# pyro-ppl/pyro

Hardware: AMD Instinct MI355X
Metric: ELBO-grad steps/sec (SVI) (higher is better)
Workload: dtype f32; 1 GPU; BASELINE configs[1]: Bayesian logistic regression, plate=1000000, D=32, Trace_ELBO num_particles=64 per GPU (vectorised), AutoNormal, Adam; full SVI.step of SVI(model, guide, optim, loss), one hipGraph replay per step; parallelism=particles sharded x1, flat RCCL grad all-reduce

## Files before the change

### include/pyro_amd.h

```cpp
#ifndef PYRO_AMD_H
#define PYRO_AMD_H

#include <stddef.h>
#include <stdint.h>

#ifdef __cplusplus
extern "C" {
#endif

#define PA_ABI_VERSION 9

enum { PA_OK = 0, PA_ERR_INVALID = -1, PA_ERR_UNSUPPORTED = -2, PA_ERR_LAUNCH = -3 };

enum { PA_F32 = 0, PA_F64 = 1 };

enum {
  PA_DIST_NORMAL = 0,
  PA_DIST_BERNOULLI_LOGITS = 1,
  PA_DIST_HALF_CAUCHY = 2,
  PA_DIST_LOG_NORMAL = 3,
  PA_DIST_EXPONENTIAL = 4,
  PA_DIST_HALF_NORMAL = 5,
  PA_DIST_GAMMA = 6,
  PA_DIST_BETA = 7,
// ... 372 lines not shown
int pa_tall_wgrad(const float* G, const float* X, int64_t B, int64_t R, int64_t K, float* dW, float* db,
                  void* workspace, size_t workspace_bytes, pa_stream_t stream);
int pa_tall_linear_act(const float* G, int64_t B, int64_t R, const float* W, int64_t w_row_stride,
                       int64_t w_col_stride, int64_t C, const float* bias, const float* y_mul,
                       int sigmoid_out, float* Y, pa_stream_t stream);
int pa_tall_wgrad_act(const float* G, const float* X, const float* y_mul, int64_t B, int64_t R, int64_t K,
                      float* dW, float* db, void* workspace, size_t workspace_bytes, pa_stream_t stream);
int pa_tall_linear_path(int64_t B, int64_t R, int64_t C, int64_t w_row_stride, int64_t w_col_stride,
                        int g_aligned16, int ymul_aligned16, int w_aligned16);
int pa_tall_wgrad_path(int64_t B, int64_t R, int64_t K);

int pa_gamma_rsample(int dtype, void* out, void* d_alpha, pa_view2d alpha, int64_t rows, int64_t cols,
                     uint64_t seed, uint64_t offset, const uint64_t* offset_dev, pa_stream_t stream);
int pa_gamma_implicit_grad(int dtype, void* d_alpha, pa_view2d alpha, pa_view2d value, int64_t rows,
                           int64_t cols, pa_stream_t stream);

#define PA_CHAIN_SYNC_BYTES 64
int pa_chain_begin(pa_stream_t stream, void* sync_words, size_t sync_bytes);
int pa_chain_flush(void);
int pa_chain_end(int* launches, int* phases);
int pa_chain_pending(void);
int pa_chain_tune(int fuse_tail);
int pa_chain_fused_launches(void);
int pa_chain_debug_stamps(void* stamps32);

#define PA_RTC_MAX_POINTERS 384
int pa_rtc_compile(const char* source, const char* kernel_name, void** function_out);
int pa_rtc_compile_cached(const char* source, const char* kernel_name, const char* cache_file,
                          void** function_out, int* compiled_out);
int pa_rtc_version(int* hiprtc_major, int* hiprtc_minor, int* runtime_version);
void* pa_rtc_blocks_begin(void);
int pa_rtc_blocks_end(void* scope, int64_t* n_blocks_out);
int pa_rtc_blocks_free(void* scope);
int pa_rtc_launch(void* function, uint32_t grid, uint32_t block, const void* const* pointers,
                  int n_pointers, pa_stream_t stream);

size_t pa_mixture_workspace(int K, int64_t B);
int pa_mixture_fwd_bwd(int dtype, int dist, const void* x, int64_t N, int K, int64_t B, const void* a,
                       int64_t a_batch_stride, const void* p0, int64_t p0_stride, int64_t p0_batch_stride,
                       const void* p1, int64_t p1_stride, int64_t p1_batch_stride, void* workspace,
                       size_t workspace_bytes, double* out, pa_stream_t stream);

int pa_mixture_diag_normal_layout(int K, int D, int* kp_out, int* dd_out);
size_t pa_mixture_diag_normal_workspace(int K, int D, int64_t B);
int pa_mixture_diag_normal_fwd_bwd(int dtype, const void* x, int64_t N, int D, int K, int64_t B, const void* a,
                                   int64_t a_batch_stride, const void* loc, int64_t loc_stride_k,
// ... 59 lines not shown
```

### pyro_amd/_lib.py

```python
import ctypes
import os
from ctypes import (POINTER, Structure, c_char_p, c_double, c_int, c_int32, c_int64, c_size_t, c_uint32,
                    c_uint64, c_void_p)

_HERE = os.path.dirname(os.path.abspath(__file__))
LIB_PATH = os.path.join(_HERE, "lib", "libpyro_amd.so")

PA_OK, PA_ERR_INVALID, PA_ERR_UNSUPPORTED, PA_ERR_LAUNCH = 0, -1, -2, -3
PA_F32, PA_F64 = 0, 1
ABI_VERSION = 9

DIST_NORMAL = 0
DIST_BERNOULLI_LOGITS = 1
DIST_HALF_CAUCHY = 2
DIST_LOG_NORMAL = 3
DIST_EXPONENTIAL = 4
DIST_HALF_NORMAL = 5
DIST_GAMMA = 6
DIST_BETA = 7
DIST_POISSON = 8
DIST_BINOMIAL_LOGITS = 9
DIST_KL_NORMAL_LOC = 10
DIST_KL_NORMAL_SCALE = 11

# ... 280 lines not shown
                                c_void_p]),
    "pa_bow_workspace": (c_size_t, [c_int64, c_int64, c_int64]),
    "pa_bow_linear_fwd": (c_int, [c_void_p, c_void_p, c_void_p, c_int64, c_int64, c_int64, c_void_p,
                                  c_void_p, c_size_t, c_void_p]),
    "pa_bow_linear_bwd": (c_int, [c_void_p, c_void_p, c_int64, c_int64, c_int64, c_void_p, c_void_p,
                                  c_size_t, c_void_p]),
    "pa_bow_linear_fwd_act": (c_int, [c_void_p, c_void_p, c_void_p, c_int64, c_int64, c_int64, c_int, c_void_p,
                                      c_void_p, c_size_t, c_void_p]),
    "pa_bow_linear_bwd_act": (c_int, [c_void_p, c_void_p, c_void_p, c_int64, c_int64, c_int64, c_void_p,
                                      c_void_p, c_void_p, c_size_t, c_void_p]),
    "pa_tsgemm_tn_workspace": (c_size_t, [c_int64, c_int64, c_int64]),
    "pa_tsgemm_tn": (c_int, [c_void_p, c_void_p, c_int64, c_int64, c_int64, c_void_p, c_void_p, c_size_t,
                             c_void_p]),
    "pa_gamma_rsample": (c_int, [c_int, c_void_p, c_void_p, View2D, c_int64, c_int64, c_uint64, c_uint64,
                                 c_void_p, c_void_p]),
    "pa_gamma_implicit_grad": (c_int, [c_int, c_void_p, View2D, View2D, c_int64, c_int64, c_void_p]),
    "pa_chain_begin": (c_int, [c_void_p, c_void_p, c_size_t]),
    "pa_chain_flush": (c_int, []),
    "pa_chain_end": (c_int, [POINTER(c_int), POINTER(c_int)]),
    "pa_chain_pending": (c_int, []),
    "pa_chain_debug_stamps": (c_int, [c_void_p]),
    "pa_chain_tune": (c_int, [c_int]),
    "pa_chain_fused_launches": (c_int, []),
    "pa_adam_step_publish": (c_int, [c_int, c_void_p, c_void_p, c_void_p, c_void_p, c_int64,
                                     c_double, c_double, c_double, c_double, c_double, c_double,
                                     c_double, c_int, c_void_p, c_int, c_int, c_void_p, c_void_p,
                                     c_void_p, c_void_p, c_uint64, c_void_p]),
}

_lib = None


def exported_symbols():
    return sorted(_SIGNATURES)


def load(path=None):
    global _lib
    if _lib is not None:
        return _lib
    path = path or os.environ.get("PYRO_AMD_LIB", LIB_PATH)
    if not os.path.exists(path):
        raise RuntimeError(
            "pyro_amd: HIP extension %s not found. Build it with "
            "`python -m pyro_amd.csrc.build` (hipcc --offload-arch=gfx950). There is no CPU "
            "fallback." % path)
# ... 24 lines not shown
```

### pyro_amd/csrc/chain.hip

```cpp
#include "chain.h"
#include "glm_finalize.h"
#include "multisite_dev.h"
#include "optim_dev.h"
#include "site_tail.h"

namespace pa {

constexpr int CH_FIN = 0, CH_MULTI = 1, CH_MF = 2, CH_ADAM = 3, CH_PHASES = 4;
constexpr int CH_MF_SITES = 8;

struct MfArgs8 {
  int nsites;
  MfSiteDev s[CH_MF_SITES];
};
static_assert(offsetof(MfArgs8, s) == offsetof(MfArgs, s), "layout");

constexpr int CH_TAIL_ENTRIES = 6;
struct TailSite {
  int n_entries;
  int entries[CH_TAIL_ENTRIES];
  int extras_mask;
  int64_t off_loc, off_rho;
  int fast;
  int layout;
// ... 7 lines not shown
  double fin_scale, fin_ll_offset;
  int fin_nblocks, fin_npass, fin_D, fin_P, fin_DT, fin_PT;
  float* multi_out;
  const float* multi_g;
  double multi_coef_all;
  int multi_accumulate, multi_n;
  int64_t mf_P;
  int mf_gy, mf_nsites;
  float *ad_p, *ad_g, *ad_m, *ad_v;
  int64_t ad_n;
  double ad_lr, ad_b1, ad_b2, ad_eps, ad_wd, ad_clip, ad_lrd;
  int64_t* ad_step;
  int ad_clipped, ad_zero;
  AdamPublish ad_pub;
  uint32_t* sync;
  int have[CH_PHASES];
  int grid[CH_PHASES];
  int last;
  uint64_t* stamps;
  const int64_t* gate;
  uint32_t jitter;
  int tail_nsites;
  uint32_t fin_dep_mask;
  TailSite tail[CH_MF_SITES];
};
static_assert(sizeof(ChainArgs) <= 6144, "kernel arguments grew unexpectedly");

__device__ __forceinline__ void chain_jitter(uint32_t seed, int p, uint32_t salt) {
  if (seed == 0u) return;
  uint32_t hsh = seed * 2654435761u ^ (blockIdx.x + 1u) * 40503u ^ (uint32_t)(p + 1) * 2246822519u ^ salt;
  hsh ^= hsh >> 15;
  hsh *= 2654435761u;
  hsh ^= hsh >> 13;
  const uint32_t n = (hsh >> 8) & 63u;
  if ((hsh & 3u) == 0u) return;
  for (uint32_t i = 0; i < n; ++i) __builtin_amdgcn_s_sleep(8);
}

__device__ __forceinline__ void chain_signal(uint32_t jitter, uint32_t* sync, int p, uint32_t expected,
                                             bool last) {
  chain_jitter(jitter, p, 0x9e3779b9u);
  __syncthreads();
  if (threadIdx.x == 0) {
    __builtin_amdgcn_fence(__ATOMIC_RELEASE, "agent");
    const uint32_t old =
        __hip_atomic_fetch_add(&sync[p], 1u, __ATOMIC_RELAXED, __HIP_MEMORY_SCOPE_AGENT);
// ... 19 lines not shown
}

template <int DT, int PT, int SUB>
__device__ __forceinline__ void chain_fin(const ChainArgs& a, int me, int nw) {
  __shared__ double sm[SUB][FIN_GROUPS][FIN_OUT];
  const int sub = SUB == 1 ? 0 : (int)(threadIdx.x >> 8), tid = (int)(threadIdx.x & 255);
  for (int64_t base = (int64_t)me * SUB; base < a.grid[CH_FIN]; base += (int64_t)nw * SUB) {
    glm_finalize_body<DT, PT>(base + sub, a.fin_part, a.fin_nblocks, a.fin_npass, a.fin_D, a.fin_P,
                              a.fin_scale, a.fin_ll, a.fin_gw, a.fin_gb, a.fin_ll_offset, tid,
                              sm[sub]);
    __syncthreads();
  }
}
template <int SUB>
__device__ __forceinline__ void chain_fin_any(const ChainArgs& a, int me, int nw) {
  if (a.fin_DT == 1 && a.fin_PT == 2) chain_fin<1, 2, SUB>(a, me, nw);
  else if (a.fin_DT == 1 && a.fin_PT == 1) chain_fin<1, 1, SUB>(a, me, nw);
  else if (a.fin_DT == 2 && a.fin_PT == 1) chain_fin<2, 1, SUB>(a, me, nw);
  else if (a.fin_DT == 2 && a.fin_PT == 2) chain_fin<2, 2, SUB>(a, me, nw);
  else if (a.fin_DT == 4 && a.fin_PT == 2) chain_fin<4, 2, SUB>(a, me, nw);
  else chain_fin<4, 1, SUB>(a, me, nw);
}

#define PA_CHAIN_STAMP(i)                                                     \
  do {                                                                        \
    if (a.stamps != nullptr && threadIdx.x == 0 && (me == 0 || total_wg))     \
      a.stamps[(total_wg ? 16 : 0) + (i)] = wall_clock64();                   \
  } while (0)

__global__ __launch_bounds__(1024) void chain_kernel(const ChainArgs a) {
  if (a.gate != nullptr && *a.gate != 0) return;
  const bool total_wg = blockIdx.x == gridDim.x - 1;
  if (!total_wg && threadIdx.x >= 256) return;
  const int nw = (int)gridDim.x - 1, me = (int)blockIdx.x;
  uint32_t* sync = a.sync;
  const int part_fin = a.grid[CH_FIN] < nw ? a.grid[CH_FIN] : nw;
  const int part_multi = (a.multi_n < nw ? a.multi_n : nw) + 1;
  const int part_mf = a.grid[CH_MF] < nw ? a.grid[CH_MF] : nw;
  int prev = -1, prev_n = 0;
  PA_CHAIN_STAMP(0);

  if (a.have[CH_FIN]) {
    if (!total_wg && me < part_fin) {
      chain_fin_any<1>(a, me, nw);
      chain_signal(a.jitter, sync, CH_FIN, (uint32_t)part_fin, a.last == CH_FIN);
    }
    prev = CH_FIN;
    prev_n = part_fin;
  }
  PA_CHAIN_STAMP(1);
  if (a.have[CH_MULTI]) {
    constexpr uint32_t KB = (uint32_t)offsetof(ChainArgs, multi);
    if (total_wg || me < part_multi - 1) {
      if (prev >= 0) chain_wait(a.jitter, sync, prev, (uint32_t)prev_n);
      PA_CHAIN_STAMP(2);
      if (total_wg) {
        multi_sum_body<float, MULTI_THREADS>(KB, a.multi_out, a.multi_coef_all, a.multi_accumulate);
      } else {
        for (int vb = me; vb < a.multi_n; vb += nw) {
          multi_grad_body<float>(KB, vb, a.multi_g, a.multi_coef_all);
          __syncthreads();
        }
      }
      chain_signal(a.jitter, sync, CH_MULTI, (uint32_t)part_multi, a.last == CH_MULTI);
    }
    prev = CH_MULTI;
    prev_n = part_multi;
  }
  PA_CHAIN_STAMP(3);
  if (total_wg) return;
  if (a.have[CH_MF]) {
    constexpr uint32_t KB = (uint32_t)offsetof(ChainArgs, mf);
    if (me < part_mf) {
      if (prev >= 0) chain_wait(a.jitter, sync, prev, (uint32_t)prev_n);
      PA_CHAIN_STAMP(4);
      for (int vb = me; vb < a.grid[CH_MF]; vb += nw) {
        meanfield_sample_bwd_body<float>(KB, (uint32_t)(vb % a.mf_nsites),
                                         (uint32_t)(vb / a.mf_nsites), (uint32_t)a.mf_gy, a.mf_P);
        __syncthreads();
      }
      chain_signal(a.jitter, sync, CH_MF, (uint32_t)part_mf, a.last == CH_MF);
    }
    prev = CH_MF;
    prev_n = part_mf;
  }
  PA_CHAIN_STAMP(5);
  if (a.have[CH_ADAM]) {
    const int part_adam = a.grid[CH_ADAM] < nw ? a.grid[CH_ADAM] : nw;
    if (me < part_adam) {
      if (prev >= 0) chain_wait(a.jitter, sync, prev, (uint32_t)prev_n);
      PA_CHAIN_STAMP(6);
      for (int64_t vb = me; vb < a.grid[CH_ADAM]; vb += nw)
        adam_body<float>(vb, (int64_t)a.grid[CH_ADAM], a.ad_p, a.ad_g, a.ad_m, a.ad_v, a.ad_n,
                         a.ad_lr, a.ad_b1, a.ad_b2, a.ad_eps, a.ad_wd, a.ad_clip, a.ad_lrd,
                         a.ad_clipped, a.ad_step, a.ad_zero, a.ad_pub);
      chain_signal(a.jitter, sync, CH_ADAM, (uint32_t)part_adam, a.last == CH_ADAM);
    }
  }
  PA_CHAIN_STAMP(7);
}

__global__ __launch_bounds__(1024) void chain_tail_kernel(const ChainArgs a) {
  if (a.gate != nullptr && *a.gate != 0) return;
  const bool total_wg = blockIdx.x == gridDim.x - 1;
  const int nw = (int)gridDim.x - 1, me = (int)blockIdx.x;
  uint32_t* sync = a.sync;
  if (me < a.tail_nsites && threadIdx.x >= 256) return;
  const int nfw = nw - a.tail_nsites;
  const int fin_vwg = (a.grid[CH_FIN] + 3) / 4;
  const int part_fin = fin_vwg < nfw ? fin_vwg : nfw;
  PA_CHAIN_STAMP(0);
  if (!total_wg && me >= a.tail_nsites) {
    const int fme = me - a.tail_nsites;
    if (a.have[CH_FIN] && fme < part_fin) {
      chain_fin_any<4>(a, fme, nfw);
      chain_signal(a.jitter, sync, CH_FIN, (uint32_t)part_fin, false);
    }
    return;
// ... 25 lines not shown
    auto wait = [&]() {
      PA_CHAIN_STAMP(7);
      if (a.have[CH_FIN]) chain_wait(a.jitter, sync, CH_FIN, (uint32_t)part_fin);
      else __syncthreads();
      PA_CHAIN_STAMP(2);
    };
    site_fast<PA_DIST_NORMAL>(eh, eg, ms, layout, a.multi_coef_all, off_loc, off_rho, ad, fast_red,
                              fast_xch, wait, &step);
    PA_CHAIN_STAMP(5);
  } else {
  double total_acc = 0.0;
  if (total_wg) {
    total_acc = multi_sum_partial<float, MULTI_THREADS>(KB, a.fin_dep_mask, 0u);
  }
  if (!total_wg) {
    ts_n = kernarg_load<int>(KT + (uint32_t)offsetof(TailSite, n_entries));
    ts_mask = kernarg_load<int>(KT + (uint32_t)offsetof(TailSite, extras_mask));
    for (int q = 0; q < ts_n; ++q) {
      multi_grad_body<float>(KB, tail_entry(q), a.multi_g, a.multi_coef_all, GRAD_NO_EXTRAS);
      __syncthreads();
    }
  }
  PA_CHAIN_STAMP(7);
  if (a.have[CH_FIN]) chain_wait(a.jitter, sync, CH_FIN, (uint32_t)part_fin);
  PA_CHAIN_STAMP(2);
  if (total_wg) {
    total_acc += multi_sum_partial<float, MULTI_THREADS>(KB, 0u, a.fin_dep_mask);
    multi_sum_finish<float>(total_acc, a.multi_out, a.multi_coef_all, a.multi_accumulate);
    if (threadIdx.x == 0) step = a.ad_step[0] + 1;
  } else {
    for (int q = 0; q < ts_n; ++q)
      if (ts_mask >> q & 1)
        multi_grad_body<float>(KB, tail_entry(q), a.multi_g, a.multi_coef_all, GRAD_EXTRAS_ONLY);
    __syncthreads();
    PA_CHAIN_STAMP(3);
    meanfield_sample_bwd_body<float>(KMF, (uint32_t)me, 0u, 1u, a.mf_P);
    __syncthreads();
    PA_CHAIN_STAMP(4);
    const MfSiteDev ms = kernarg_load<MfSiteDev>(KMF + (uint32_t)offsetof(MfArgs, s) +
                                                 (uint32_t)me * (uint32_t)sizeof(MfSiteDev));
    const int64_t off_loc = kernarg_load<int64_t>(KT + (uint32_t)offsetof(TailSite, off_loc));
    const int64_t off_rho = kernarg_load<int64_t>(KT + (uint32_t)offsetof(TailSite, off_rho));
    adam_two_ranges<float>(off_loc, off_rho, ms.n, a.ad_p, a.ad_g, a.ad_m, a.ad_v, a.ad_step,
                           a.ad_lr, a.ad_b1, a.ad_b2, a.ad_eps, a.ad_wd, a.ad_clip, a.ad_lrd,
                           a.ad_clipped, a.ad_zero, &step);
    PA_CHAIN_STAMP(5);
  }
  }
  __syncthreads();
  if (threadIdx.x == 0) {
    __builtin_amdgcn_fence(__ATOMIC_RELEASE, "agent");
    const unsigned long long ticket = __hip_atomic_fetch_add(
        reinterpret_cast<unsigned long long*>(a.ad_step + 1), 1ull, __ATOMIC_RELAXED,
        __HIP_MEMORY_SCOPE_AGENT);
    if (ticket == (unsigned long long)a.tail_nsites) {
      __builtin_amdgcn_fence(__ATOMIC_ACQUIRE, "agent");
      a.ad_step[1] = 0;
      a.ad_step[0] = step;
#pragma unroll
      for (int q = 0; q < CH_PHASES; ++q)
        __hip_atomic_store(&sync[q], 0u, __ATOMIC_RELAXED, __HIP_MEMORY_SCOPE_AGENT);
      publish_to_host(a.ad_pub);
    }
  }
  PA_CHAIN_STAMP(6);
}

static int g_chain_fast_sites = 1;

static bool chain_plan_tail(ChainArgs& a) {
  if (!(a.have[CH_MULTI] && a.have[CH_MF] && a.have[CH_ADAM])) return false;
  if (a.multi_g != nullptr || a.mf_nsites < 1 || a.mf_nsites > CH_MF_SITES) return false;
  const float* g0 = a.ad_g;
  const float* g1 = a.ad_g + a.ad_n;
  int owner[PA_MULTI_MAX_ENTRIES];
  for (int e = 0; e < a.multi.n; ++e) owner[e] = -1;
  int64_t covered = 0;
  int64_t lo[2 * CH_MF_SITES], hi[2 * CH_MF_SITES];
  for (int k = 0; k < a.mf_nsites; ++k) {
    const MfSiteDev& s = a.mf.s[k];
    TailSite& t = a.tail[k];
    t.n_entries = 0;
    t.extras_mask = 0;
    if (s.n < 1 || s.n > 4096 || !s.accumulate || s.d_loc == nullptr || s.d_rho == nullptr) return false;
    const float* dl = (const float*)s.d_loc;
    const float* dr = (const float*)s.d_rho;
    if (dl < g0 || dl + s.n > g1 || dr < g0 || dr + s.n > g1) return false;
    t.off_loc = dl - g0;
    t.off_rho = dr - g0;
    lo[2 * k] = t.off_loc; hi[2 * k] = t.off_loc + s.n;
    lo[2 * k + 1] = t.off_rho; hi[2 * k + 1] = t.off_rho + s.n;
// ... 32 lines not shown
        found = en.dv == w || en.da == w || en.db == w;
      }
      if (!found) return false;
    }
  }
  if (covered != a.ad_n) return false;
  const int m = 2 * a.mf_nsites;
  for (int i = 0; i < m; ++i)
    for (int j = i + 1; j < m; ++j)
      if (lo[i] < hi[j] && lo[j] < hi[i]) return false;
  a.fin_dep_mask = 0u;
  if (a.have[CH_FIN]) {
    auto in_fin = [&](const void* p) {
      const float* f = (const float*)p;
      return p != nullptr &&
             ((f >= a.fin_ll && f < a.fin_ll + a.fin_P) || (f >= a.fin_gb && f < a.fin_gb + a.fin_P) ||
              (f >= a.fin_gw && f < a.fin_gw + (int64_t)a.fin_P * a.fin_D));
    };
    for (int e = 0; e < a.multi.n; ++e) {
      const EntryDev& en = a.multi.e[e];
      if (in_fin(en.v) || in_fin(en.a) || in_fin(en.b) || in_fin(en.m)) a.fin_dep_mask |= 1u << e;
    }
    if (a.multi.n > MULTI_THREADS / 64) a.fin_dep_mask = 0xffffffffu;
  }
  for (int k = 0; k < a.mf_nsites; ++k) {
    const MfSiteDev& s = a.mf.s[k];
    TailSite& t = a.tail[k];
    t.fast = 0;
    t.layout = SITE_LAYOUT_COLS;
    if (!g_chain_fast_sites || t.n_entries != 2) continue;
    const EntryDev& h = a.multi.e[t.entries[0]];
    const EntryDev& q = a.multi.e[t.entries[1]];
    const bool family = h.dist == PA_DIST_NORMAL;
    const bool shape =
        family && q.dist == PA_DIST_NORMAL && h.m == nullptr &&
        q.m == nullptr && h.chain_next == t.entries[1] && q.chain_next < 0 &&
        (h.need & PA_NEED_VALUE) && !(h.need & PA_VALUE_BY_CHAIN) && h.dv == s.d_z &&
        !((h.need & PA_NEED_P0) && h.da) && !((h.need & PA_NEED_P1) && h.db) &&
        (q.need & PA_VALUE_BY_CHAIN) && (q.need & PA_NEED_P0) && (q.need & PA_NEED_P1) &&
        q.da == s.d_loc_out && q.db == s.d_scale && q.da != nullptr && q.db != nullptr &&
        q.v == h.v && q.vsr == h.vsr && q.vsc == h.vsc && q.rows == h.rows && q.cols == h.cols &&
        s.d_z != nullptr && s.eps != nullptr && s.rho != nullptr;
    if (!shape) continue;
    const int64_t P = a.mf_P;
    if (s.n >= 2 && s.n <= GRAD_THREADS && h.rows == P && h.cols == s.n && h.vsr == s.n &&
        h.vsc == 1 && q.asr == 0 && q.asc == 1 && q.bsr == 0 && q.bsc == 1) {
// ... 2 lines not shown
    } else if (s.n == 1 && h.rows == 1 && h.cols == P && P >= 2 && P <= 64 && h.vsc == 1 &&
               q.asc == 0 && q.bsc == 0) {
      t.fast = 1;
      t.layout = SITE_LAYOUT_SCALAR;
    }
  }
  a.tail_nsites = a.mf_nsites;
  return true;
}

struct ChainState {
  bool on = false;
  hipStream_t stream = nullptr;
  int top = -1;
  int launches = 0;
  int phases = 0;
  int fused = 0;
  ChainArgs a;
};
static ChainState g_chain;
static uint64_t* g_chain_stamps = nullptr;
static int g_chain_fuse = 1;
static uint32_t g_chain_jitter = 0;

static int chain_launch() {
  ChainState& c = g_chain;
  if (c.top < 0) return PA_OK;
  ChainArgs& a = c.a;
  int maxgrid = 1, np = 0;
  for (int p = 0; p < CH_PHASES; ++p)
    if (a.have[p]) {
      a.last = p;
      ++np;
      if (a.grid[p] > maxgrid) maxgrid = a.grid[p];
    }
  a.stamps = g_chain_stamps;
  gate_emit_deferred(c.stream);
  a.gate = gate_word();
  a.jitter = g_chain_jitter;
  gate_aware_launch();
  int nw = cu_count() - 1;
  if (nw < 1) nw = 1;
  if (maxgrid < nw) nw = maxgrid;
  const hipStream_t s = c.stream;
  c.top = -1;
  a.tail_nsites = 0;
  if (g_chain_fuse && cu_count() - 1 > CH_MF_SITES && chain_plan_tail(a)) {
    nw = a.tail_nsites + (a.have[CH_FIN] ? (a.grid[CH_FIN] + 3) / 4 : 0);
    if (nw > cu_count() - 1) nw = cu_count() - 1;
    hipLaunchKernelGGL(chain_tail_kernel, dim3((unsigned)nw + 1), dim3(1024), 0, s, a);
    c.fused += 1;
  } else {
    hipLaunchKernelGGL(chain_kernel, dim3((unsigned)nw + 1), dim3(1024), 0, s, a);
  }
  c.launches += 1;
  c.phases += np;
  for (int p = 0; p < CH_PHASES; ++p) a.have[p] = 0;
  return check_launch("chain_kernel");
}

static bool chain_open(pa_stream_t stream, int k, int* rc) {
  ChainState& c = g_chain;
  *rc = PA_OK;
  if (!c.on) return false;
  if ((hipStream_t)stream != c.stream) {
    *rc = chain_launch();
    return false;
  }
  if (c.top >= k) *rc = chain_launch();
  if (*rc != PA_OK) return false;
  if (c.top < 0) {
    for (int p = 0; p < CH_PHASES; ++p) c.a.have[p] = 0, c.a.grid[p] = 0;
  }
  c.top = k;
  c.a.have[k] = 1;
  return true;
}
// ... 158 lines not shown
  int rc = pa::chain_flush_draw();
  if (rc != PA_OK) return rc;
  return pa::chain_launch();
}

int pa_chain_end(int* launches, int* phases) {
  int rc = PA_OK;
  if (pa::g_chain.on) {
    rc = pa::chain_flush_draw();
    const int rc2 = pa::chain_launch();
    if (rc == PA_OK) rc = rc2;
  }
  pa::g_chain.on = false;
  if (launches) *launches = pa::g_chain.launches;
  if (phases) *phases = pa::g_chain.phases;
  return rc;
}

int pa_chain_tune(int fuse_tail) {
  pa::g_chain_fuse = (fuse_tail & 1) ? 1 : 0;
  pa::g_chain_fast_sites = (fuse_tail & 2) ? 0 : 1;
  pa::g_chain_jitter = (uint32_t)fuse_tail >> 8;
  pa::g_draw_enabled = (fuse_tail & 4) ? 0 : 1;
  return PA_OK;
}

int pa_chain_fused_launches(void) { return pa::g_chain.fused; }

int pa_chain_debug_stamps(void* stamps32) {
  pa::g_chain_stamps = (uint64_t*)stamps32;
#ifdef PA_CHAIN_LATENCY_PROBE
  uint64_t* p = (uint64_t*)stamps32;
  int zero = 0;
  (void)hipMemcpyToSymbol(HIP_SYMBOL(pa::pa_dbg_stamps), &p, sizeof(p));
  (void)hipMemcpyToSymbol(HIP_SYMBOL(pa::pa_dbg_next), &zero, sizeof(zero));
#endif
  return PA_OK;
}

int pa_chain_pending(void) {
  if (!pa::g_chain.on || pa::g_chain.top < 0) return 0;
  int n = 0;
  for (int p = 0; p < pa::CH_PHASES; ++p) n += pa::g_chain.a.have[p];
  return n;
}

}
```

### pyro_amd/csrc/glm_finalize.h

```cpp
#pragma once
#include "common.h"

namespace pa {

template <int DT, int PT>
constexpr int glm_record_floats() { return PT * DT * 1024 + 2 * PT * 32; }

constexpr int FIN_OUT = 8, FIN_GROUPS = 32;
template <int DT, int PT>
__device__ __forceinline__ void glm_finalize_body(
    int64_t vb, const float* __restrict__ part, int nblocks, int npass, int D, int P, double scale,
    float* __restrict__ ll, float* __restrict__ gw, float* __restrict__ gb, double ll_offset, int tid,
    double (*sm)[FIN_OUT]) {
  constexpr int REC = glm_record_floats<DT, PT>();
  const int jj = tid % FIN_OUT, s = tid / FIN_OUT;
  const int64_t J = (int64_t)P * D + 2 * P;
  const int64_t j = vb * FIN_OUT + jj;
  double acc = 0.0;
  if (j < J) {
    int p, slot;
    if (j < (int64_t)P * D) {
      p = (int)(j / D);
      const int d = (int)(j % D);
      const int pl = p % (32 * PT), pt = pl >> 5, i = pl & 31, dt = d >> 5, c = d & 31;
      const int hh = (i >> 2) & 1, reg = (i & 3) + 4 * (i >> 3);
      slot = ((pt * DT + dt) * 16 + reg) * 64 + c + 32 * hh;
    } else {
      const int64_t k = j - (int64_t)P * D;
      const int which = k >= P ? 1 : 0;
      p = (int)(k - (int64_t)which * P);
      const int pl = p % (32 * PT), pt = pl >> 5, i = pl & 31;
      slot = PT * DT * 1024 + (2 * pt + which) * 32 + i;
    }
    const int pass = p / (32 * PT);
    const float* base = part + (int64_t)pass * nblocks * REC + slot;
    int blk = s;
    {
      float v[24];
      for (; blk + 23 * FIN_GROUPS < nblocks; blk += 24 * FIN_GROUPS) {
#pragma unroll
        for (int u = 0; u < 24; ++u) v[u] = base[(int64_t)(blk + u * FIN_GROUPS) * REC];
#pragma unroll
        for (int u = 0; u < 24; ++u) acc += (double)v[u];
      }
    }
#ifndef PA_FIN_NO16
    {
      float v[16];
      for (; blk + 15 * FIN_GROUPS < nblocks; blk += 16 * FIN_GROUPS) {
#pragma unroll
        for (int u = 0; u < 16; ++u) v[u] = base[(int64_t)(blk + u * FIN_GROUPS) * REC];
#pragma unroll
        for (int u = 0; u < 16; ++u) acc += (double)v[u];
      }
    }
#endif
    float v[8];
    for (; blk + 7 * FIN_GROUPS < nblocks; blk += 8 * FIN_GROUPS) {
#pragma unroll
      for (int u = 0; u < 8; ++u) v[u] = base[(int64_t)(blk + u * FIN_GROUPS) * REC];
#pragma unroll
      for (int u = 0; u < 8; ++u) acc += (double)v[u];
    }
    for (; blk < nblocks; blk += FIN_GROUPS) acc += (double)base[(int64_t)blk * REC];
  }
  sm[s][jj] = acc;
  __syncthreads();
  if (s == 0 && j < J) {
    double t = 0.0;
#pragma unroll
    for (int k = 0; k < FIN_GROUPS; ++k) t += sm[k][jj];
    const float v = (float)(t * scale);
    if (j < (int64_t)P * D) gw[j] = v;
    else if (j < (int64_t)P * D + P) ll[j - (int64_t)P * D] = (float)((t + ll_offset) * scale);
    else gb[j - (int64_t)P * D - P] = v;
  }
}

template <int DT, int PT>
__global__ __launch_bounds__(FIN_OUT * FIN_GROUPS) void glm_finalize_kernel(
    const float* __restrict__ part, int nblocks, int npass, int D, int P, double scale,
    float* __restrict__ ll, float* __restrict__ gw, float* __restrict__ gb, double ll_offset) {
  __shared__ double sm[FIN_GROUPS][FIN_OUT];
  glm_finalize_body<DT, PT>((int64_t)blockIdx.x, part, nblocks, npass, D, P, scale, ll, gw, gb,
                            ll_offset, (int)threadIdx.x, sm);
}

}
```

### pyro_amd/csrc/multisite_dev.h

```cpp
#pragma once
#include "common.h"
#include "dist_fam.h"

namespace pa {

struct EntryDev {
  int dist, need;
  int64_t rows, cols;
  const void *v, *a, *b;
  const uint8_t* m;
  int64_t vsr, vsc, asr, asc, bsr, bsc, msr, msc;
  double coef;
  void *dv, *da, *db;
  int chain_next;
  const void* xg;
  double xcoef;
};
struct MultiArgs {
  int n;
  EntryDev e[PA_MULTI_MAX_ENTRIES];
};

template <typename S>
__device__ __forceinline__ S kernarg_load(uint32_t byte_offset) {
// ... 97 lines not shown
template <typename T, int NTHREADS>
__device__ __forceinline__ double multi_sum_partial(uint32_t kbase, uint32_t skip_mask,
                                                    uint32_t only_mask) {
  const int n_entries = kernarg_load<int>(kbase + offsetof(MultiArgs, n));
  const int wave = __builtin_amdgcn_readfirstlane(threadIdx.x >> 6), lane = threadIdx.x & 63;
  constexpr int NW = NTHREADS / 64;
  const int wpe = n_entries >= NW ? 1 : NW / (n_entries > 0 ? n_entries : 1);
  const int epr = NW / wpe;
  double acc = 0.0;
  for (int k0 = 0; k0 < n_entries; k0 += epr) {
    const int k = k0 + wave / wpe;
    if (k < n_entries && wave / wpe < epr) {
      if ((skip_mask >> k & 1u) || (only_mask != 0u && !(only_mask >> k & 1u))) continue;
      const EntryDev e = kernarg_load<EntryDev>(kbase + offsetof(MultiArgs, e) + k * sizeof(EntryDev));
      const uint32_t tid = (uint32_t)((wave % wpe) * 64 + lane), nth = (uint32_t)(wpe * 64);
      double s = 0.0;
      PA_DISPATCH_ENTRY(e.dist, s = (entry_sum<D_, T>(e, tid, nth)));
      acc += e.coef * s;
    }
  }
  return acc;
}
template <typename T>
__device__ __forceinline__ void multi_sum_finish(double acc, T* __restrict__ out, double coef_all,
                                                 int accumulate) {
  __shared__ double smem[16];
  const double t = block_sum_f64(acc, smem);
  if (threadIdx.x == 0) {
    const double base = accumulate ? (double)*out : 0.0;
    *out = (T)(base + coef_all * t);
  }
}
template <typename T, int NTHREADS>
__device__ __forceinline__ void multi_sum_body(uint32_t kbase, T* __restrict__ out, double coef_all,
                                               int accumulate) {
  multi_sum_finish<T>(multi_sum_partial<T, NTHREADS>(kbase, 0u, 0u), out, coef_all, accumulate);
}

template <typename T>
__global__ __launch_bounds__(MULTI_THREADS) void multi_sum_kernel(const MultiArgs args_by_value,
                                                                  T* __restrict__ out,
                                                                  double coef_all, int accumulate) {
  multi_sum_body<T, MULTI_THREADS>(0u, out, coef_all, accumulate);
}

constexpr int GRAD_THREADS = 256;
__device__ __forceinline__ uint32_t row_groups(uint32_t tk) {
  const uint32_t ng = GRAD_THREADS / tk;
  return ng > 8u ? 8u : ng;
}
enum { PAT_SKIP = 0, PAT_FULL = 1, PAT_ROWRED = 2, PAT_SCALAR = 3, PAT_COLRED = 4 };
__device__ __forceinline__ int pattern_of(bool wanted, int64_t sr, int64_t sc, int64_t R, int64_t C) {
  if (!wanted) return PAT_SKIP;
  const bool red_r = (sr == 0 && R > 1), red_c = (sc == 0 && C > 1);
  return red_r ? (red_c ? PAT_SCALAR : PAT_ROWRED) : (red_c ? PAT_COLRED : PAT_FULL);
}

template <int DIST, typename T>
__device__ __forceinline__ void combined_pass(const EntryDev& e, double w, int pv, bool accumulate,
// ... 509 lines not shown
```

### pyro_amd/csrc/optim_dev.h

```cpp
#pragma once
#include "common.h"

namespace pa {

struct AdamPublish {
  const void* src;
  int src_dtype;
  double* host_value;
  uint64_t* host_seq;
  uint64_t* counter;
  uint64_t inc;
};

__device__ __forceinline__ void publish_to_host(const AdamPublish& pub) {
  uint64_t seq = 0;
  if (pub.counter != nullptr) {
    const uint64_t c0 = pub.counter[0], c1 = pub.counter[1];
    pub.counter[0] = c0 + pub.inc;
    if (pub.src != nullptr) pub.counter[1] = seq = c1 + 1;
  }
  if (pub.src != nullptr) {
    const double v = pub.src_dtype == PA_F32 ? (double)*static_cast<const float*>(pub.src)
                                             : *static_cast<const double*>(pub.src);
    __hip_atomic_store(pub.host_value, v, __ATOMIC_RELAXED, __HIP_MEMORY_SCOPE_SYSTEM);
    __threadfence_system();
    if (pub.counter == nullptr)
      seq = __hip_atomic_load(pub.host_seq, __ATOMIC_RELAXED, __HIP_MEMORY_SCOPE_SYSTEM) + 1;
    __hip_atomic_store(pub.host_seq, seq, __ATOMIC_RELEASE, __HIP_MEMORY_SCOPE_SYSTEM);
  }
}

struct AdamStep {
  double bc1, bc2, lr_t;
};
__device__ __forceinline__ double pow_int(double b, int64_t n) {
  double r = 1.0, x = b;
  while (n > 0) {
    if (n & 1) r *= x;
    x *= x;
    n >>= 1;
  }
  return r;
}
__device__ __forceinline__ AdamStep adam_step_scalars(int64_t step, double lr, double b1, double b2,
                                                      double lrd, int clipped) {
  AdamStep s;
  s.bc1 = 1.0 - pow_int(b1, step);
  s.bc2 = 1.0 - pow_int(b2, step);
  s.lr_t = clipped ? lr * pow_int(lrd, step) : lr;
  return s;
}

// ... 65 lines not shown
    adam_update<T>(ga, pa_, ma, va, st, b1, b2, eps, wd, clip, clipped);
    m[i0] = ma; v[i0] = va; p[i0] = pa_;
    adam_update<T>(gb, pb, mb, vb, st, b1, b2, eps, wd, clip, clipped);
    m[i1] = mb; v[i1] = vb; p[i1] = pb;
    if (zero_grad) { g[i0] = T(0); g[i1] = T(0); }
  }
  for (int64_t k = t + 256; k < n; k += 256) {
    for (int h = 0; h < 2; ++h) {
      const int64_t i = (h == 0 ? o0 : o1) + k;
      T pi = p[i], mi = m[i], vi = v[i];
      adam_update<T>(g[i], pi, mi, vi, st, b1, b2, eps, wd, clip, clipped);
      m[i] = mi; v[i] = vi; p[i] = pi;
      if (zero_grad) g[i] = T(0);
    }
  }
}

template <typename T>
__device__ __forceinline__ void adam_body(int64_t vb, int64_t nvb, T* __restrict__ p,
                                          T* __restrict__ g, T* __restrict__ m, T* __restrict__ v,
                                          int64_t n, double lr, double b1, double b2, double eps,
                                          double wd, double clip, double lrd, int clipped,
                                          int64_t* __restrict__ step_dev, int zero_grad,
                                          const AdamPublish& pub) {
  int64_t step;
  adam_range<T>(vb * 256 + threadIdx.x, nvb * 256, n, p, g, m, v, step_dev, lr, b1, b2, eps, wd, clip,
                lrd, clipped, zero_grad, &step);
  __syncthreads();
  if (threadIdx.x == 0) {
    bool last = true;
    if (nvb > 1) {
      const unsigned long long ticket =
          atomicAdd(reinterpret_cast<unsigned long long*>(step_dev + 1), 1ull);
      last = ticket == (unsigned long long)nvb - 1;
      if (last) step_dev[1] = 0;
    }
    if (last) {
      step_dev[0] = step;
      publish_to_host(pub);
    }
  }
}

template <typename T>
__global__ __launch_bounds__(256) void adam_kernel(T* __restrict__ p, T* __restrict__ g,
                                                   T* __restrict__ m, T* __restrict__ v, int64_t n,
                                                   double lr, double b1, double b2, double eps,
                                                   double wd, double clip, double lrd, int clipped,
                                                   int64_t* __restrict__ step_dev,
                                                   int zero_grad, AdamPublish pub) {
  adam_body<T>((int64_t)blockIdx.x, (int64_t)gridDim.x, p, g, m, v, n, lr, b1, b2, eps, wd, clip, lrd,
               clipped, step_dev, zero_grad, pub);
}

}
```

### pyro_amd/infer/svi.py

```python
import os as _os
import warnings

import torch
import torch.utils._python_dispatch

from .. import kernels, poutine
from ..params import _PARAM_STORE
from ..util import capture_scope, torch_isnan, zero_grads
from .elbo import ELBO


def _arg_key(x):
    if isinstance(x, torch.Tensor):
        return ("t", x.data_ptr(), tuple(x.shape), tuple(x.stride()), x.dtype, x.device)
    if isinstance(x, (list, tuple)):
        return tuple(_arg_key(v) for v in x)
    try:
        hash(x)
        return ("p", x)
    except TypeError:
        return ("id", id(x))


def _fast_geometry(args):
# ... 422 lines not shown
            kernels.glm_planes_revalidate()
            kernels.lda_index_revalidate()
            kernels.bow_revalidate()
            entry.cap.before_replay()
            entry.replay()
            if entry.graph2 is not None:
                entry.between()
                entry.graph2.replay()
            entry.cap.after_replay()
            if entry.eager_params is not None:
                self._update_eagerly(entry.eager_params)
            if not kwargs:
                self._last_fast = (args, _fast_geometry(args), entry)
            return entry.read_loss()
        return self._gated_step(entry, args, kwargs)

    def _update_eagerly(self, params):
        self.optim(params)
        if not getattr(self.optim, "zeroes_grads", False):
            grads = [p.grad for p in params if p.grad is not None]
            if grads:
                torch._foreach_zero_(grads)

    def _drop(self, key):
        e = self._graphs.pop(key, None)
        if e is not None:
            e.alive = False
        return e

    def release(self):
        for e in self._graphs.values():
            if e.armed:
                e.cancel()
            e.alive = False
        self._armed_fast = self._last_fast = None
        self._graphs.clear()
        self._const_rec.clear()

    def pause(self):
        self._armed_fast = None
        for e in self._graphs.values():
            if e.armed:
                e.cancel()

    def disarm(self):
        self.prearm = False
        self._armed_fast = None
        for e in self._graphs.values():
            if e.armed:
                e.cancel()
            e.arm_backoff = 1 << 60

    def _host_state(self, args, kwargs, entry=None):
        from .. import rng
        refs = [(t, t._version) for t in entry.reads] if entry is not None else []
        for a in list(args) + [v for _, v in sorted(kwargs.items())]:
            if isinstance(a, torch.Tensor):
# ... 202 lines not shown
```

### pyro_amd/kernels.py

```python
import ctypes
import os

import torch
import torch.utils._python_dispatch

from . import _lib
from ._lib import NULL_VIEW, Unsupported, View2D, check

_DTYPES = {torch.float32: _lib.PA_F32, torch.float64: _lib.PA_F64}


def on_device(t):
    return t.is_cuda


def _require_gpu(*tensors):
    for t in tensors:
        if t is not None and not t.is_cuda:
            raise RuntimeError(
                "pyro_amd: kernel called with a tensor on %s; the HIP backend only runs on an "
                "MI355X device and has no CPU fallback" % t.device)


def _dtype(t):
# ... 124 lines not shown
    def __torch_dispatch__(self, func, types, args=(), kwargs=None):
        if not _launches_nothing(func):
            if "torch_ops" in _CHAIN:
                _CHAIN["torch_ops"] += 1
            chain_flush()
        return func(*args, **(kwargs or {}))


def chain_sync_buffer(device):
    device = torch.device(device)
    key = (device.type, device.index if device.index is not None else torch.cuda.current_device())
    buf = _CHAIN["sync"].get(key)
    if buf is None:
        buf = torch.zeros((_lib.CHAIN_SYNC_BYTES // 4,), dtype=torch.int32, device=device)
        _CHAIN["sync"][key] = buf
    return buf


def chain_debug_stamps(buf):
    check(_lib.load().pa_chain_debug_stamps(None if buf is None else ctypes.c_void_p(buf.data_ptr())))
    _CHAIN["stamps"] = buf


def chain_tune(fuse_tail=True, fast_sites=True, jitter_seed=0, fuse_draw=True):
    check(_lib.load().pa_chain_tune((1 if fuse_tail else 0) | (0 if fast_sites else 2)
                                    | (0 if fuse_draw else 4) | ((int(jitter_seed) & 0x7fffff) << 8)))


def chain_flush():
    if _CHAIN["keep"] is not None:
        check(_lib.load().pa_chain_flush())


class chain_recording:

    def __init__(self, device):
        self.sync = chain_sync_buffer(device)
        self.stats = (0, 0)
        self.fused = 0
        self._guard = None

    def __enter__(self):
        assert _CHAIN["keep"] is None, "nested chain recordings"
        check(_lib.load().pa_chain_begin(_stream(), ctypes.c_void_p(self.sync.data_ptr()),
                                         self.sync.numel() * 4))
        _CHAIN["keep"] = []
        self._guard = _ChainGuard()
        self._guard.__enter__()
        return self
# ... 1931 lines not shown
```

Baseline: 13620 ELBO-grad steps/s (64 particles x 1e6-row plate per step).

## Publish the loss to the host before Adam finishes in the fused chain kernel

Adds an early hand-over path to the fused chain kernel. The ELBO loss is written to the host-visible value and sequence word as soon as the multi-site sum produces it, and the Adam tail then does only counter bookkeeping. This aims to let the host read the loss and move on without waiting for the optimizer phase to finish. It also adds an opt-in, off-by-default path where the tail workgroup computes the log-likelihood reduction itself instead of waiting on the finalize phase, and factors the finalize reduction into shared helpers. Graph drop and release now synchronize the stream, which adds host stalls on those rare paths.

```diff
diff --git a/include/pyro_amd.h b/include/pyro_amd.h
--- a/include/pyro_amd.h
+++ b/include/pyro_amd.h
@@ -418,6 +418,7 @@
 int pa_chain_pending(void);
 int pa_chain_tune(int fuse_tail);
 int pa_chain_fused_launches(void);
+int pa_chain_last_form(int* form4);
 int pa_chain_debug_stamps(void* stamps32);
 
 #define PA_RTC_MAX_POINTERS 384
diff --git a/pyro_amd/_lib.py b/pyro_amd/_lib.py
--- a/pyro_amd/_lib.py
+++ b/pyro_amd/_lib.py
@@ -326,6 +326,7 @@
     "pa_chain_debug_stamps": (c_int, [c_void_p]),
     "pa_chain_tune": (c_int, [c_int]),
     "pa_chain_fused_launches": (c_int, []),
+    "pa_chain_last_form": (c_int, [POINTER(c_int)]),
     "pa_adam_step_publish": (c_int, [c_int, c_void_p, c_void_p, c_void_p, c_void_p, c_int64,
                                      c_double, c_double, c_double, c_double, c_double, c_double,
                                      c_double, c_int, c_void_p, c_int, c_int, c_void_p, c_void_p,
diff --git a/pyro_amd/csrc/chain.hip b/pyro_amd/csrc/chain.hip
--- a/pyro_amd/csrc/chain.hip
+++ b/pyro_amd/csrc/chain.hip
@@ -53,6 +53,8 @@
   uint32_t jitter;
   int tail_nsites;
   uint32_t fin_dep_mask;
+  int early;
+  int fin_direct_ll;
   TailSite tail[CH_MF_SITES];
 };
 static_assert(sizeof(ChainArgs) <= 6144, "kernel arguments grew unexpectedly");
@@ -118,6 +120,41 @@
   else chain_fin<4, 1, SUB>(a, me, nw);
 }
 
+constexpr int LL_NB = 2;
+__device__ __forceinline__ void chain_ll_direct(const ChainArgs& a, double (*sm)[FIN_GROUPS][32]) {
+  const int jj = (int)(threadIdx.x & 31), s = (int)(threadIdx.x >> 5);
+  const int DT = a.fin_DT, PT = a.fin_PT, P = a.fin_P;
+  const int rec = PT * DT * 1024 + 2 * PT * 32;
+  for (int p0 = 0; p0 < P; p0 += 32 * LL_NB) {
+    const float* base[LL_NB];
+    double acc[LL_NB];
+#pragma unroll
+    for (int o = 0; o < LL_NB; ++o) {
+      const int p = p0 + 32 * o + jj < P ? p0 + 32 * o + jj : 0;
+      base[o] = glm_fin_base(a.fin_part, DT, PT, a.fin_nblocks, rec, p, glm_fin_vec_slot(DT, PT, p, 0));
+      acc[o] = 0.0;
+    }
+    glm_fin_group_sum<LL_NB, 16>(base, s, a.fin_nblocks, rec, acc);
+#pragma unroll
+    for (int o = 0; o < LL_NB; ++o) sm[o][s][jj] = acc[o];
+    __syncthreads();
+    if (s < LL_NB) {
+      const int p = p0 + 32 * s + jj;
+      if (p < P)
+        a.fin_ll[p] = glm_fin_ll_value(glm_fin_combine(&sm[s][0][jj], 32), a.fin_ll_offset, a.fin_scale);
+    }
+    __syncthreads();
+  }
+}
+
+#define PA_CHAIN_HAND_OVER(loss)                                \
+  do {                                                          \
+    if (a.early && threadIdx.x == 0) {                          \
+      publish_hand_over(a.ad_pub, (double)(loss));              \
+      PA_CHAIN_STAMP(8);                                        \
+    }                                                           \
+  } while (0)
+
 #define PA_CHAIN_STAMP(i)                                                     \
   do {                                                                        \
     if (a.stamps != nullptr && threadIdx.x == 0 && (me == 0 || total_wg))     \
@@ -151,7 +188,9 @@
       if (prev >= 0) chain_wait(a.jitter, sync, prev, (uint32_t)prev_n);
       PA_CHAIN_STAMP(2);
       if (total_wg) {
-        multi_sum_body<float, MULTI_THREADS>(KB, a.multi_out, a.multi_coef_all, a.multi_accumulate);
+        const float loss = multi_sum_body<float, MULTI_THREADS>(KB, a.multi_out, a.multi_coef_all,
+                                                                a.multi_accumulate);
+        PA_CHAIN_HAND_OVER(loss);
       } else {
         for (int vb = me; vb < a.multi_n; vb += nw) {
           multi_grad_body<float>(KB, vb, a.multi_g, a.multi_coef_all);
@@ -189,7 +228,7 @@
       for (int64_t vb = me; vb < a.grid[CH_ADAM]; vb += nw)
         adam_body<float>(vb, (int64_t)a.grid[CH_ADAM], a.ad_p, a.ad_g, a.ad_m, a.ad_v, a.ad_n,
                          a.ad_lr, a.ad_b1, a.ad_b2, a.ad_eps, a.ad_wd, a.ad_clip, a.ad_lrd,
-                         a.ad_clipped, a.ad_step, a.ad_zero, a.ad_pub);
+                         a.ad_clipped, a.ad_step, a.ad_zero, a.ad_pub, a.early != 0);
       chain_signal(a.jitter, sync, CH_ADAM, (uint32_t)part_adam, a.last == CH_ADAM);
     }
   }
@@ -261,11 +300,18 @@
     }
   }
   PA_CHAIN_STAMP(7);
-  if (a.have[CH_FIN]) chain_wait(a.jitter, sync, CH_FIN, (uint32_t)part_fin);
+  if (total_wg && a.fin_direct_ll) {
+    __shared__ double ll_sm[LL_NB][FIN_GROUPS][32];
+    chain_ll_direct(a, ll_sm);
+  } else if (a.have[CH_FIN]) {
+    chain_wait(a.jitter, sync, CH_FIN, (uint32_t)part_fin);
+  }
   PA_CHAIN_STAMP(2);
   if (total_wg) {
     total_acc += multi_sum_partial<float, MULTI_THREADS>(KB, 0u, a.fin_dep_mask);
-    multi_sum_finish<float>(total_acc, a.multi_out, a.multi_coef_all, a.multi_accumulate);
+    const float loss =
+        multi_sum_finish<float>(total_acc, a.multi_out, a.multi_coef_all, a.multi_accumulate);
+    PA_CHAIN_HAND_OVER(loss);
     if (threadIdx.x == 0) step = a.ad_step[0] + 1;
   } else {
     for (int q = 0; q < ts_n; ++q)
@@ -299,13 +345,16 @@
 #pragma unroll
       for (int q = 0; q < CH_PHASES; ++q)
         __hip_atomic_store(&sync[q], 0u, __ATOMIC_RELAXED, __HIP_MEMORY_SCOPE_AGENT);
-      publish_to_host(a.ad_pub);
+      if (a.early) publish_bookkeeping(a.ad_pub);
+      else publish_to_host(a.ad_pub);
     }
   }
   PA_CHAIN_STAMP(6);
 }
 
 static int g_chain_fast_sites = 1;
+static int g_chain_early = 1;
+static int g_chain_direct_ll = 0;
 
 static bool chain_plan_tail(ChainArgs& a) {
   if (!(a.have[CH_MULTI] && a.have[CH_MF] && a.have[CH_ADAM])) return false;
@@ -384,6 +433,16 @@
       if (in_fin(en.v) || in_fin(en.a) || in_fin(en.b) || in_fin(en.m)) a.fin_dep_mask |= 1u << e;
     }
     if (a.multi.n > MULTI_THREADS / 64) a.fin_dep_mask = 0xffffffffu;
+    bool other = false;
+    for (int e = 0; e < a.multi.n; ++e) {
+      const EntryDev& en = a.multi.e[e];
+      const void* reads[4] = {en.v, en.a, en.b, en.m};
+      for (const void* p : reads) {
+        const float* f = (const float*)p;
+        if (in_fin(p) && !(f >= a.fin_ll && f < a.fin_ll + a.fin_P)) other = true;
+      }
+    }
+    a.fin_direct_ll = a.early && g_chain_direct_ll && a.fin_dep_mask != 0u && !other && a.fin_nblocks > 0;
   }
   for (int k = 0; k < a.mf_nsites; ++k) {
     const MfSiteDev& s = a.mf.s[k];
@@ -432,6 +491,7 @@
 static uint64_t* g_chain_stamps = nullptr;
 static int g_chain_fuse = 1;
 static uint32_t g_chain_jitter = 0;
+static int g_chain_last_form[4] = {0, 0, 0, 0};
 
 static int chain_launch() {
   ChainState& c = g_chain;
@@ -455,6 +515,9 @@
   const hipStream_t s = c.stream;
   c.top = -1;
   a.tail_nsites = 0;
+  a.early = g_chain_early && a.have[CH_MULTI] && a.have[CH_ADAM] && a.ad_pub.src != nullptr &&
+            a.ad_pub.src == (const void*)a.multi_out && a.ad_pub.src_dtype == PA_F32;
+  a.fin_direct_ll = 0;
   if (g_chain_fuse && cu_count() - 1 > CH_MF_SITES && chain_plan_tail(a)) {
     nw = a.tail_nsites + (a.have[CH_FIN] ? (a.grid[CH_FIN] + 3) / 4 : 0);
     if (nw > cu_count() - 1) nw = cu_count() - 1;
@@ -463,6 +526,10 @@
   } else {
     hipLaunchKernelGGL(chain_kernel, dim3((unsigned)nw + 1), dim3(1024), 0, s, a);
   }
+  g_chain_last_form[0] = a.early;
+  g_chain_last_form[1] = a.fin_direct_ll;
+  g_chain_last_form[2] = a.have[CH_FIN] ? a.fin_nblocks : 0;
+  g_chain_last_form[3] = a.have[CH_FIN] ? a.fin_npass : 0;
   c.launches += 1;
   c.phases += np;
   for (int p = 0; p < CH_PHASES; ++p) a.have[p] = 0;
@@ -667,10 +734,18 @@
   pa::g_chain_fast_sites = (fuse_tail & 2) ? 0 : 1;
   pa::g_chain_jitter = (uint32_t)fuse_tail >> 8;
   pa::g_draw_enabled = (fuse_tail & 4) ? 0 : 1;
+  pa::g_chain_early = (fuse_tail & 8) ? 0 : 1;
+  pa::g_chain_direct_ll = (fuse_tail & 16) ? 1 : 0;
   return PA_OK;
 }
 
 int pa_chain_fused_launches(void) { return pa::g_chain.fused; }
+
+int pa_chain_last_form(int* form4) {
+  PA_REQUIRE(form4 != nullptr, "pa_chain_last_form: NULL output");
+  for (int i = 0; i < 4; ++i) form4[i] = pa::g_chain_last_form[i];
+  return PA_OK;
+}
 
 int pa_chain_debug_stamps(void* stamps32) {
   pa::g_chain_stamps = (uint64_t*)stamps32;
diff --git a/pyro_amd/csrc/glm_finalize.h b/pyro_amd/csrc/glm_finalize.h
--- a/pyro_amd/csrc/glm_finalize.h
+++ b/pyro_amd/csrc/glm_finalize.h
@@ -6,7 +6,93 @@
 template <int DT, int PT>
 constexpr int glm_record_floats() { return PT * DT * 1024 + 2 * PT * 32; }
 
-constexpr int FIN_OUT = 8, FIN_GROUPS = 32;
+__device__ __forceinline__ int glm_fin_vec_slot(int DT, int PT, int p, int which) {
+  const int pl = p % (32 * PT), pt = pl >> 5, i = pl & 31;
+  return PT * DT * 1024 + (2 * pt + which) * 32 + i;
+}
+__device__ __forceinline__ int glm_fin_slot(int DT, int PT, int64_t j, int D, int P, int* p_out) {
+  if (j < (int64_t)P * D) {
+    const int p = (int)(j / D);
+    const int d = (int)(j % D);
+    const int pl = p % (32 * PT), pt = pl >> 5, i = pl & 31, dt = d >> 5, c = d & 31;
+    const int hh = (i >> 2) & 1, reg = (i & 3) + 4 * (i >> 3);
+    *p_out = p;
+    return ((pt * DT + dt) * 16 + reg) * 64 + c + 32 * hh;
+  }
+  const int64_t k = j - (int64_t)P * D;
+  const int which = k >= P ? 1 : 0;
+  *p_out = (int)(k - (int64_t)which * P);
+  return glm_fin_vec_slot(DT, PT, *p_out, which);
+}
+__device__ __forceinline__ const float* glm_fin_base(const float* __restrict__ part, int DT, int PT,
+                                                     int nblocks, int rec, int p, int slot) {
+  const int pass = p / (32 * PT);
+  return part + (int64_t)pass * nblocks * rec + slot;
+}
+
+constexpr int FIN_GROUPS = 32;
+template <int NB, int MAXB = 24>
+__device__ __forceinline__ void glm_fin_group_sum(const float* const (&base)[NB], int s, int nblocks,
+                                                  int rec, double (&acc)[NB]) {
+  int blk = s;
+  if constexpr (MAXB >= 24) {
+    float v[NB][24];
+    for (; blk + 23 * FIN_GROUPS < nblocks; blk += 24 * FIN_GROUPS) {
+#pragma unroll
+      for (int o = 0; o < NB; ++o)
+#pragma unroll
+        for (int u = 0; u < 24; ++u) v[o][u] = base[o][(int64_t)(blk + u * FIN_GROUPS) * rec];
+#pragma unroll
+      for (int o = 0; o < NB; ++o)
+#pragma unroll
+        for (int u = 0; u < 24; ++u) acc[o] += (double)v[o][u];
+    }
+  }
+#ifndef PA_FIN_NO16
+  {
+    float v[NB][16];
+    for (; blk + 15 * FIN_GROUPS < nblocks; blk += 16 * FIN_GROUPS) {
+#pragma unroll
+      for (int o = 0; o < NB; ++o)
+#pragma unroll
+        for (int u = 0; u < 16; ++u) v[o][u] = base[o][(int64_t)(blk + u * FIN_GROUPS) * rec];
+#pragma unroll
+      for (int o = 0; o < NB; ++o)
+#pragma unroll
+        for (int u = 0; u < 16; ++u) acc[o] += (double)v[o][u];
+    }
+  }
+#endif
+  float v[NB][8];
+  for (; blk + 7 * FIN_GROUPS < nblocks; blk += 8 * FIN_GROUPS) {
+#pragma unroll
+    for (int o = 0; o < NB; ++o)
+#pragma unroll
+      for (int u = 0; u < 8; ++u) v[o][u] = base[o][(int64_t)(blk + u * FIN_GROUPS) * rec];
+#pragma unroll
+    for (int o = 0; o < NB; ++o)
+#pragma unroll
+      for (int u = 0; u < 8; ++u) acc[o] += (double)v[o][u];
+  }
+  for (; blk < nblocks; blk += FIN_GROUPS) {
+    float w[NB];
+#pragma unroll
+    for (int o = 0; o < NB; ++o) w[o] = base[o][(int64_t)blk * rec];
+#pragma unroll
+    for (int o = 0; o < NB; ++o) acc[o] += (double)w[o];
+  }
+}
+__device__ __forceinline__ double glm_fin_combine(const double* sm, int stride) {
+  double t = 0.0;
+#pragma unroll
+  for (int k = 0; k < FIN_GROUPS; ++k) t += sm[k * stride];
+  return t;
+}
+__device__ __forceinline__ float glm_fin_ll_value(double t, double ll_offset, double scale) {
+  return (float)((t + ll_offset) * scale);
+}
+
+constexpr int FIN_OUT = 8;
 template <int DT, int PT>
 __device__ __forceinline__ void glm_finalize_body(
     int64_t vb, const float* __restrict__ part, int nblocks, int npass, int D, int P, double scale,
@@ -16,63 +102,20 @@
   const int jj = tid % FIN_OUT, s = tid / FIN_OUT;
   const int64_t J = (int64_t)P * D + 2 * P;
   const int64_t j = vb * FIN_OUT + jj;
-  double acc = 0.0;
+  double acc[1] = {0.0};
   if (j < J) {
-    int p, slot;
-    if (j < (int64_t)P * D) {
-      p = (int)(j / D);
-      const int d = (int)(j % D);
-      const int pl = p % (32 * PT), pt = pl >> 5, i = pl & 31, dt = d >> 5, c = d & 31;
-      const int hh = (i >> 2) & 1, reg = (i & 3) + 4 * (i >> 3);
-      slot = ((pt * DT + dt) * 16 + reg) * 64 + c + 32 * hh;
-    } else {
-      const int64_t k = j - (int64_t)P * D;
-      const int which = k >= P ? 1 : 0;
-      p = (int)(k - (int64_t)which * P);
-      const int pl = p % (32 * PT), pt = pl >> 5, i = pl & 31;
-      slot = PT * DT * 1024 + (2 * pt + which) * 32 + i;
-    }
-    const int pass = p / (32 * PT);
-    const float* base = part + (int64_t)pass * nblocks * REC + slot;
-    int blk = s;
-    {
-      float v[24];
-      for (; blk + 23 * FIN_GROUPS < nblocks; blk += 24 * FIN_GROUPS) {
-#pragma unroll
-        for (int u = 0; u < 24; ++u) v[u] = base[(int64_t)(blk + u * FIN_GROUPS) * REC];
-#pragma unroll
-        for (int u = 0; u < 24; ++u) acc += (double)v[u];
-      }
-    }
-#ifndef PA_FIN_NO16
-    {
-      float v[16];
-      for (; blk + 15 * FIN_GROUPS < nblocks; blk += 16 * FIN_GROUPS) {
-#pragma unroll
-        for (int u = 0; u < 16; ++u) v[u] = base[(int64_t)(blk + u * FIN_GROUPS) * REC];
-#pragma unroll
-        for (int u = 0; u < 16; ++u) acc += (double)v[u];
-      }
-    }
-#endif
-    float v[8];
-    for (; blk + 7 * FIN_GROUPS < nblocks; blk += 8 * FIN_GROUPS) {
-#pragma unroll
-      for (int u = 0; u < 8; ++u) v[u] = base[(int64_t)(blk + u * FIN_GROUPS) * REC];
-#pragma unroll
-      for (int u = 0; u < 8; ++u) acc += (double)v[u];
-    }
-    for (; blk < nblocks; blk += FIN_GROUPS) acc += (double)base[(int64_t)blk * REC];
+    int p;
+    const int slot = glm_fin_slot(DT, PT, j, D, P, &p);
+    const float* const base[1] = {glm_fin_base(part, DT, PT, nblocks, REC, p, slot)};
+    glm_fin_group_sum<1>(base, s, nblocks, REC, acc);
   }
-  sm[s][jj] = acc;
+  sm[s][jj] = acc[0];
   __syncthreads();
   if (s == 0 && j < J) {
-    double t = 0.0;
-#pragma unroll
-    for (int k = 0; k < FIN_GROUPS; ++k) t += sm[k][jj];
+    const double t = glm_fin_combine(&sm[0][jj], FIN_OUT);
     const float v = (float)(t * scale);
     if (j < (int64_t)P * D) gw[j] = v;
-    else if (j < (int64_t)P * D + P) ll[j - (int64_t)P * D] = (float)((t + ll_offset) * scale);
+    else if (j < (int64_t)P * D + P) ll[j - (int64_t)P * D] = glm_fin_ll_value(t, ll_offset, scale);
     else gb[j - (int64_t)P * D - P] = v;
   }
 }
diff --git a/pyro_amd/csrc/multisite_dev.h b/pyro_amd/csrc/multisite_dev.h
--- a/pyro_amd/csrc/multisite_dev.h
+++ b/pyro_amd/csrc/multisite_dev.h
@@ -143,19 +143,22 @@
   return acc;
 }
 template <typename T>
-__device__ __forceinline__ void multi_sum_finish(double acc, T* __restrict__ out, double coef_all,
-                                                 int accumulate) {
+__device__ __forceinline__ T multi_sum_finish(double acc, T* __restrict__ out, double coef_all,
+                                              int accumulate) {
   __shared__ double smem[16];
   const double t = block_sum_f64(acc, smem);
+  T r = T(0);
   if (threadIdx.x == 0) {
     const double base = accumulate ? (double)*out : 0.0;
-    *out = (T)(base + coef_all * t);
-  }
+    r = (T)(base + coef_all * t);
+    *out = r;
+  }
+  return r;
 }
 template <typename T, int NTHREADS>
-__device__ __forceinline__ void multi_sum_body(uint32_t kbase, T* __restrict__ out, double coef_all,
-                                               int accumulate) {
-  multi_sum_finish<T>(multi_sum_partial<T, NTHREADS>(kbase, 0u, 0u), out, coef_all, accumulate);
+__device__ __forceinline__ T multi_sum_body(uint32_t kbase, T* __restrict__ out, double coef_all,
+                                            int accumulate) {
+  return multi_sum_finish<T>(multi_sum_partial<T, NTHREADS>(kbase, 0u, 0u), out, coef_all, accumulate);
 }
 
 template <typename T>
diff --git a/pyro_amd/csrc/optim_dev.h b/pyro_amd/csrc/optim_dev.h
--- a/pyro_amd/csrc/optim_dev.h
+++ b/pyro_amd/csrc/optim_dev.h
@@ -12,22 +12,24 @@
   uint64_t inc;
 };
 
+__device__ __forceinline__ void publish_hand_over(const AdamPublish& pub, double v) {
+  if (pub.src == nullptr) return;
+  uint64_t seq = 0;
+  if (pub.counter != nullptr) pub.counter[1] = seq = pub.counter[1] + 1;
+  __hip_atomic_store(pub.host_value, v, __ATOMIC_RELAXED, __HIP_MEMORY_SCOPE_SYSTEM);
+  __threadfence_system();
+  if (pub.counter == nullptr)
+    seq = __hip_atomic_load(pub.host_seq, __ATOMIC_RELAXED, __HIP_MEMORY_SCOPE_SYSTEM) + 1;
+  __hip_atomic_store(pub.host_seq, seq, __ATOMIC_RELEASE, __HIP_MEMORY_SCOPE_SYSTEM);
+}
+__device__ __forceinline__ void publish_bookkeeping(const AdamPublish& pub) {
+  if (pub.counter != nullptr) pub.counter[0] = pub.counter[0] + pub.inc;
+}
 __device__ __forceinline__ void publish_to_host(const AdamPublish& pub) {
-  uint64_t seq = 0;
-  if (pub.counter != nullptr) {
-    const uint64_t c0 = pub.counter[0], c1 = pub.counter[1];
-    pub.counter[0] = c0 + pub.inc;
-    if (pub.src != nullptr) pub.counter[1] = seq = c1 + 1;
-  }
-  if (pub.src != nullptr) {
-    const double v = pub.src_dtype == PA_F32 ? (double)*static_cast<const float*>(pub.src)
-                                             : *static_cast<const double*>(pub.src);
-    __hip_atomic_store(pub.host_value, v, __ATOMIC_RELAXED, __HIP_MEMORY_SCOPE_SYSTEM);
-    __threadfence_system();
-    if (pub.counter == nullptr)
-      seq = __hip_atomic_load(pub.host_seq, __ATOMIC_RELAXED, __HIP_MEMORY_SCOPE_SYSTEM) + 1;
-    __hip_atomic_store(pub.host_seq, seq, __ATOMIC_RELEASE, __HIP_MEMORY_SCOPE_SYSTEM);
-  }
+  publish_bookkeeping(pub);
+  if (pub.src != nullptr)
+    publish_hand_over(pub, pub.src_dtype == PA_F32 ? (double)*static_cast<const float*>(pub.src)
+                                                   : *static_cast<const double*>(pub.src));
 }
 
 struct AdamStep {
@@ -139,7 +141,7 @@
                                           int64_t n, double lr, double b1, double b2, double eps,
                                           double wd, double clip, double lrd, int clipped,
                                           int64_t* __restrict__ step_dev, int zero_grad,
-                                          const AdamPublish& pub) {
+                                          const AdamPublish& pub, bool handed_over = false) {
   int64_t step;
   adam_range<T>(vb * 256 + threadIdx.x, nvb * 256, n, p, g, m, v, step_dev, lr, b1, b2, eps, wd, clip,
                 lrd, clipped, zero_grad, &step);
@@ -154,7 +156,8 @@
     }
     if (last) {
       step_dev[0] = step;
-      publish_to_host(pub);
+      if (handed_over) publish_bookkeeping(pub);
+      else publish_to_host(pub);
     }
   }
 }
diff --git a/pyro_amd/infer/svi.py b/pyro_amd/infer/svi.py
--- a/pyro_amd/infer/svi.py
+++ b/pyro_amd/infer/svi.py
@@ -468,9 +468,15 @@
             if grads:
                 torch._foreach_zero_(grads)
 
+    @staticmethod
+    def _quiesce():
+        if torch.cuda.is_available() and torch.cuda.is_initialized():
+            torch.cuda.current_stream().synchronize()
+
     def _drop(self, key):
         e = self._graphs.pop(key, None)
         if e is not None:
+            self._quiesce()
             e.alive = False
         return e
 
@@ -479,6 +485,8 @@
             if e.armed:
                 e.cancel()
             e.alive = False
+        if self._graphs:
+            self._quiesce()
         self._armed_fast = self._last_fast = None
         self._graphs.clear()
         self._const_rec.clear()
diff --git a/pyro_amd/kernels.py b/pyro_amd/kernels.py
--- a/pyro_amd/kernels.py
+++ b/pyro_amd/kernels.py
@@ -170,9 +170,17 @@
     _CHAIN["stamps"] = buf
 
 
-def chain_tune(fuse_tail=True, fast_sites=True, jitter_seed=0, fuse_draw=True):
+def chain_tune(fuse_tail=True, fast_sites=True, jitter_seed=0, fuse_draw=True, early_handover=True,
+               direct_ll=False):
     check(_lib.load().pa_chain_tune((1 if fuse_tail else 0) | (0 if fast_sites else 2)
-                                    | (0 if fuse_draw else 4) | ((int(jitter_seed) & 0x7fffff) << 8)))
+                                    | (0 if fuse_draw else 4) | (0 if early_handover else 8) | (16 if direct_ll else 0)
+                                    | ((int(jitter_seed) & 0x7fffff) << 8)))
+
+
+def chain_last_form():
+    out = (ctypes.c_int * 4)()
+    check(_lib.load().pa_chain_last_form(out))
+    return {"early": bool(out[0]), "direct_ll": bool(out[1]), "records": out[2], "passes": out[3]}
 
 
 def chain_flush():
```

Measured after the change: 13720 ELBO-grad steps/s (64 particles x 1e6-row plate per step), median of 2. Within noise of the previous version (+0.7%).
